# ChrisTho23/DrakeGPT

Hardware: NVIDIA B200
Metric: train_tokens_per_sec_TransformerLM_scaled (higher is better)
Workload: dtype bf16

## Files before the change

drakegpt_b200/csrc/attn_tc.cu:

```cuda
#include <cuda.h>

#include "common.cuh"
#include "ptx.cuh"

namespace dgpt {

using namespace ptx;

int make_tmap_bf16_2d(CUtensorMap* map, const void* base, int64_t inner, int64_t outer, int64_t ld, int box_outer);

static constexpr int HD = 64;
static constexpr int QT = 128;
static constexpr float kLog2e = 1.4426950408889634f;

struct AttnTcP {
  void *o, *dq, *dk, *dv;
  const void *o_in, *d_o;
  float* lse;
  int64_t o_rs, dq_rs, dk_rs, dv_rs, do_rs;
  int B, NH, T;
  float scale, inv_keep;
  uint32_t thr, site;
  uint64_t seed;
  const uint64_t* seed_dev;
};

__device__ __forceinline__ uint32_t pack_bf16(float a, float b) {
  __nv_bfloat162 v = __floats2bfloat162_rn(a, b);
  return *reinterpret_cast<uint32_t*>(&v);
}

__device__ __forceinline__ void store_row32_sw128(uint8_t* tile_base, int row, int c0, const float (&v)[32]) {
  uint8_t* blk = tile_base + (c0 >> 6) * 16384 + row * 128;
  const int chunk0 = (c0 & 63) >> 3;
#pragma unroll
  for (int j = 0; j < 4; ++j) {
    uint4 w;
    w.x = pack_bf16(v[8 * j], v[8 * j + 1]);
    w.y = pack_bf16(v[8 * j + 2], v[8 * j + 3]);
    w.z = pack_bf16(v[8 * j + 4], v[8 * j + 5]);
    w.w = pack_bf16(v[8 * j + 6], v[8 * j + 7]);
    *reinterpret_cast<uint4*>(blk + (((chunk0 + j) ^ (row & 7)) << 4)) = w;
  }
}

static constexpr int kFwd2Threads = 320;
static constexpr int kFwd2QK = 49152;
static constexpr int kFwd2Smem = 2 * kFwd2QK + 2 * 32768 + 256 + 1024;
static constexpr int kWHeavy = 5, kWLight = 2;

struct FwdSched {
  int nheavy, nlight;
  unsigned long long* probe;
};

__global__ void __launch_bounds__(kFwd2Threads, 1)
attn_fwd_tc2_kernel(const __grid_constant__ CUtensorMap map_q32, const __grid_constant__ CUtensorMap map_k,
                    const __grid_constant__ CUtensorMap map_v, AttnTcP p, FwdSched sc) {
  extern __shared__ uint8_t smem_raw[];
  uint8_t* smem = reinterpret_cast<uint8_t*>((reinterpret_cast<uintptr_t>(smem_raw) + 1023) & ~(uintptr_t)1023);
  uint8_t* sQK = smem;
  uint8_t* sV = smem + 2 * kFwd2QK;
  uint64_t* bars = reinterpret_cast<uint64_t*>(sV + 2 * 32768);
  uint64_t *qk_full = bars, *qk_empty = bars + 2, *v_full = bars + 4, *v_empty = bars + 6, *s_full = bars + 8,
           *p_full = bars + 10, *o_full = bars + 12, *slot_free = bars + 14;
  uint32_t* tmem_slot = reinterpret_cast<uint32_t*>(bars + 16);

  clock_probe_begin(sc.probe);
  const int warp = threadIdx.x >> 5, lane = threadIdx.x & 31;
  const int ntile = p.T / QT;

  const int G = gridDim.x, c = blockIdx.x;
  const int hq = sc.nheavy / G, hr = sc.nheavy % G;
  const int nh_c = hq + (c < hr ? 1 : 0);
  const int U = (kWHeavy * sc.nheavy + kWLight * sc.nlight + G - 1) / G;
  const int cap_hi = max(0, (U - kWHeavy * (hq + 1)) / kWLight), cap_lo = max(0, (U - kWHeavy * hq) / kWLight);
  const int cap_total = hr * cap_hi + (G - hr) * cap_lo;
  const int l_start = c < hr ? c * cap_hi : hr * cap_hi + (c - hr) * cap_lo;
  const int l0 = min(sc.nlight, l_start), l1 = min(sc.nlight, l_start + (c < hr ? cap_hi : cap_lo));
  const int n_extra = cap_total < sc.nlight ? (sc.nlight - cap_total - c + G - 1) / G : 0;
  const int n_items = nh_c + (l1 - l0) + max(0, n_extra);
  auto item = [&](int n, int& bh, int& qt) {
    if (n < nh_c) {
      const int hi = c + n * G;
      bh = hi; qt = ntile - 1;
    } else {
      const int m = n - nh_c;
      const int li = m < l1 - l0 ? l0 + m : cap_total + c + (m - (l1 - l0)) * G;
      bh = li; qt = 0;
    }
  };

  if (threadIdx.x == 0) {
    prefetch_tensormap(&map_q32);
    prefetch_tensormap(&map_k);
    prefetch_tensormap(&map_v);
    for (int g = 0; g < 2; ++g) {
      mbar_init(&qk_full[g], 1);
      mbar_init(&qk_empty[g], 1);
      mbar_init(&v_full[g], 1);
      mbar_init(&v_empty[g], 1);
      mbar_init(&s_full[g], 1);
      mbar_init(&p_full[g], 4);
      mbar_init(&o_full[g], 1);
      mbar_init(&slot_free[g], 4);
    }
    fence_barrier_init();
  }
  if (warp == 9) tmem_alloc<512>(tmem_slot);
  tc_fence_before();
  __syncthreads();
  tc_fence_after();
  const uint32_t tmem = *tmem_slot;
  pdl_grid_sync();

  if (warp == 8) {
    for (int n = 0; n < n_items; ++n) {
      const int g = n & 1, k = n >> 1;
      int bh, qt;
      item(n, bh, qt);
      const int nkv = qt + 1, b = bh / p.NH, h = bh % p.NH, row0 = b * p.T;
      uint8_t* q_s = sQK + g * kFwd2QK;
      uint8_t* v_s = sV + g * 32768;
      mbar_wait(&qk_empty[g], (k & 1) ^ 1);
      if (elect_one()) {
        mbar_expect_tx(&qk_full[g], 16384 * (1 + nkv));
        for (int qb = 0; qb < 4; ++qb)
          tma_load_2d(q_s + qb * 4096, &map_q32, &qk_full[g], h * HD, row0 + qt * QT + (g ? 3 - qb : qb) * 32);
        for (int j = 0; j < nkv; ++j) tma_load_2d(q_s + 16384 * (1 + j), &map_k, &qk_full[g], h * HD, row0 + j * QT);
      }
      __syncwarp();
      mbar_wait(&v_empty[g], (k & 1) ^ 1);
      if (elect_one()) {
        mbar_expect_tx(&v_full[g], 16384 * nkv);
        for (int kb = 0; kb < 2 * nkv; ++kb) tma_load_2d(v_s + kb * 8192, &map_v, &v_full[g], h * HD, row0 + kb * 64);
      }
      __syncwarp();
    }
  } else if (warp == 9) {
    constexpr uint32_t idesc_s = make_idesc_bf16(128, 128, 0, 0);
    constexpr uint32_t idesc_o = make_idesc_bf16(128, 64, 0, 1);
    int next_s = 0, next_pv = 0;
    while (next_pv < n_items) {
      bool progressed = false;
      if (next_s < n_items) {
        const int g = next_s & 1, k = next_s >> 1;
        if (mbar_test(&qk_full[g], k & 1) && mbar_test(&slot_free[g], (k & 1) ^ 1)) {
          tc_fence_after();
          int bh, qt;
          item(next_s, bh, qt);
          const int nkv = qt + 1;
          const uint64_t dq0 = make_smem_desc_sw128(smem_u32(sQK + g * kFwd2QK), 16, 1024);
          const uint64_t dk0 = make_smem_desc_sw128(smem_u32(sQK + g * kFwd2QK + 16384), 16, 1024);
          if (elect_one()) {
            for (int j = 0; j < nkv; ++j) {
#pragma unroll
              for (int kk = 0; kk < 4; ++kk)
                tc_mma_bf16(tmem + g * 256 + j * 128, dq0 + (uint64_t)(kk * 2), dk0 + (uint64_t)(j * 1024 + kk * 2), idesc_s, kk > 0);
            }
            tc_commit(&s_full[g]);
            tc_commit(&qk_empty[g]);
          }
          __syncwarp();
          ++next_s;
          progressed = true;
        }
      }
      if (next_pv < next_s) {
        const int g = next_pv & 1, k = next_pv >> 1;
        if (mbar_test(&p_full[g], k & 1) && mbar_test(&v_full[g], k & 1)) {
          tc_fence_after();
          int bh, qt;
          item(next_pv, bh, qt);
          const int nkv = qt + 1;
          const uint64_t dv0 = make_smem_desc_sw128(smem_u32(sV + g * 32768), 8192, 1024);
          if (elect_one()) {
            for (int kb = 0; kb < 2 * nkv; ++kb) {
#pragma unroll
              for (int kk = 0; kk < 4; ++kk)
                tc_mma_bf16_ts(tmem + g * 256 + nkv * 64, tmem + g * 256 + kb * 32 + kk * 8, dv0 + (uint64_t)(kb * 512 + kk * 128),
                               idesc_o, (kb | kk) > 0);
            }
            tc_commit(&o_full[g]);
            tc_commit(&v_empty[g]);
          }
          __syncwarp();
          ++next_pv;
          progressed = true;
        }
      }
      if (!progressed) __nanosleep(32);
    }
  } else {
    const int g = warp >> 2;
    const int quad = warp & 3;
    const int rblk = g ? 3 - quad : quad;
    const int row = rblk * 32 + lane;
    const uint32_t taddr = tmem + (uint32_t)(g * 256) + ((uint32_t)(quad * 32) << 16);
    uint64_t seed = p.seed;
    if (p.thr && p.seed_dev) seed += *p.seed_dev;
    const float sc2 = p.scale * kLog2e;
    for (int n = g; n < n_items; n += 2) {
      const int k = n >> 1;
      int bh, qt;
      item(n, bh, qt);
      const int nkv = qt + 1, b = bh / p.NH, h = bh % p.NH, row0 = b * p.T;
      const int qg = qt * QT + row;
      const int ncols = nkv * QT;
#define FTS(i) do { if (sc.probe && blockIdx.x == 0 && warp == 0 && lane == 0 && k < 3) sc.probe[4 + k * 8 + (i)] = (unsigned long long)clock64(); } while (0)
      FTS(0);
      mbar_wait(&s_full[g], k & 1);
      FTS(1);
      tc_fence_after();
      const int qg_max = qt * QT + rblk * 32 + 31, qg_min = qt * QT + rblk * 32;
      float mx = -INFINITY;
      for (int cc = 0; cc < ncols && cc <= qg_max; cc += 32) {
        uint32_t r[32];
        tmem_ld32(taddr + cc, r);
        tmem_ld_wait();
        if (cc + 31 <= qg_min) {
#pragma unroll
          for (int j = 0; j < 32; ++j) mx = fmaxf(mx, __uint_as_float(r[j]));
        } else {
#pragma unroll
          for (int j = 0; j < 32; ++j)
            if (cc + j <= qg) mx = fmaxf(mx, __uint_as_float(r[j]));
        }
      }
      FTS(2);
      const float msc = mx * sc2;
      float sum = 0.f;
      const uint64_t base = (((uint64_t)b * p.NH + h) * p.T + qg) * (uint64_t)p.T;
      for (int cc = 0; cc < ncols; cc += 32) {
        float e[32];
        if (cc > qg_max) {
#pragma unroll
          for (int j = 0; j < 32; ++j) e[j] = 0.f;
        } else {
          uint32_t r[32];
          tmem_ld32(taddr + cc, r);
          tmem_ld_wait();
          if (cc + 31 <= qg_min) {
#pragma unroll
            for (int j = 0; j < 32; ++j) {
              const float v = exp2f(__uint_as_float(r[j]) * sc2 - msc);
              sum += v;
              e[j] = v;
            }
          } else {
#pragma unroll
            for (int j = 0; j < 32; ++j) {
              const float v = (cc + j <= qg) ? exp2f(__uint_as_float(r[j]) * sc2 - msc) : 0.f;
              sum += v;
              e[j] = v;
            }
          }
          if (p.thr) {
            const DropGroup dg = dropout_group(seed, p.site, (base + cc) >> 5);
#pragma unroll
            for (int j = 0; j < 32; ++j)
              if (dropout_word(dg, j) < p.thr) e[j] = 0.f;
          }
        }
        uint32_t pk[16];
#pragma unroll
        for (int j = 0; j < 16; ++j) pk[j] = pack_bf16(e[2 * j], e[2 * j + 1]);
        tmem_st16(taddr + (cc >> 1), pk);
      }
      if (p.lse) p.lse[((int64_t)b * p.NH + h) * p.T + qg] = mx * p.scale + logf(sum);
      tmem_st_wait();
      tc_fence_before();
      __syncwarp();
      if (lane == 0) mbar_arrive(&p_full[g]);
      FTS(3);
      mbar_wait(&o_full[g], k & 1);
      FTS(4);
      tc_fence_after();
      const float oscale = p.inv_keep / sum;
      __nv_bfloat16* orow = reinterpret_cast<__nv_bfloat16*>(p.o) + (int64_t)(row0 + qg) * p.o_rs + h * HD;
#pragma unroll
      for (int cc = 0; cc < HD; cc += 32) {
        uint32_t r[32];
        tmem_ld32(taddr + nkv * 64 + cc, r);
        tmem_ld_wait();
#pragma unroll
        for (int j = 0; j < 4; ++j) {
          uint4 w;
          w.x = pack_bf16(__uint_as_float(r[8 * j]) * oscale, __uint_as_float(r[8 * j + 1]) * oscale);
          w.y = pack_bf16(__uint_as_float(r[8 * j + 2]) * oscale, __uint_as_float(r[8 * j + 3]) * oscale);
          w.z = pack_bf16(__uint_as_float(r[8 * j + 4]) * oscale, __uint_as_float(r[8 * j + 5]) * oscale);
          w.w = pack_bf16(__uint_as_float(r[8 * j + 6]) * oscale, __uint_as_float(r[8 * j + 7]) * oscale);
          *reinterpret_cast<uint4*>(orow + cc + 8 * j) = w;
        }
      }
      tc_fence_before();
      __syncwarp();
      if (lane == 0) mbar_arrive(&slot_free[g]);
      FTS(5);
    }
  }
  tc_fence_before();
  __syncthreads();
  if (warp == 9) {
    tc_fence_after();
    tmem_dealloc<512>(tmem);
  }
  clock_probe_end(sc.probe);
}

#ifdef DGPT_ATTN_TS
__device__ long long g_attn_ts[64];
#endif
static constexpr int kBwdThreads = 64 + 256;
static constexpr int kBwdSmem = 8 * 16384 + 2 * 32768 + 16384 + 2048 + 1024 + 128;

template <bool DIAG, bool DROP>
__device__ __forceinline__ void bwd_chunk_math(const AttnTcP& p, uint32_t lane_addr_st, uint32_t lane_addr_dp, int row, int k0,
                                               float sc, float lse2, float Dq, uint64_t seed, uint64_t base,
                                               float (&pd)[32], float (&ds)[32]) {
  uint32_t st[32], dp[32];
  tmem_ld32(lane_addr_st + k0, st);
  tmem_ld32(lane_addr_dp + k0, dp);
  tmem_ld_wait();
  DropGroup g = {0u, 0u};
  if (DROP) g = dropout_group(seed, p.site, (base + k0) >> 5);
#pragma unroll
  for (int t = 0; t < 32; ++t) {
    float pv = exp2f(__uint_as_float(st[t]) * sc - lse2);
    if (DIAG) pv = (k0 + t) <= row ? pv : 0.f;
    float dpv = __uint_as_float(dp[t]);
    float pdv = pv;
    if (DROP) {
      const bool keep = dropout_word(g, t) >= p.thr;
      dpv = keep ? dpv * p.inv_keep : 0.f;
      pdv = keep ? pv * p.inv_keep : 0.f;
    }
    pd[t] = pdv;
    ds[t] = pv * (dpv - Dq) * p.scale;
  }
}

template <bool DROP>
__global__ void __launch_bounds__(kBwdThreads, 1)
attn_bwd_tc_kernel(const __grid_constant__ CUtensorMap map_q, const __grid_constant__ CUtensorMap map_k,
                   const __grid_constant__ CUtensorMap map_v, const __grid_constant__ CUtensorMap map_do,
                   const __grid_constant__ CUtensorMap map_o, const __grid_constant__ CUtensorMap map_dq,
                   const __grid_constant__ CUtensorMap map_dk, const __grid_constant__ CUtensorMap map_dv, AttnTcP p) {
  extern __shared__ __align__(1024) uint8_t smem[];
  uint8_t* sQ = smem;
  uint8_t* sK = smem + 2 * 16384;
  uint8_t* sV = smem + 4 * 16384;
  uint8_t* sG = smem + 6 * 16384;
  uint8_t* sPd = smem + 8 * 16384;
  uint8_t* sDs = sPd + 32768;
  uint8_t* sSt = sDs + 32768;
  float* lse_s = reinterpret_cast<float*>(sSt + 16384);
  float* D_s = lse_s + 256;
  uint64_t* bars = reinterpret_cast<uint64_t*>(D_s + 256);
  uint64_t *ld_a = bars, *st_full = bars + 1, *ps_full = bars + 2, *drained = bars + 3, *acc_done = bars + 4;
  uint64_t *ld_b = bars + 5, *ld_c = bars + 6;
  uint64_t* acc_free = bars + 7;
  uint32_t* tmem_slot = reinterpret_cast<uint32_t*>(bars + 8);

  const int warp = threadIdx.x >> 5, lane = threadIdx.x & 31;
#ifdef DGPT_ATTN_TS
#define BTS(i) do { if (blockIdx.x == 0 && blockIdx.y == (gridDim.y / 2) && warp == 2 && lane == 0) g_attn_ts[i] = clock64(); } while (0)
#else
#define BTS(i) do { } while (0)
#endif
  BTS(0);
  const int h = blockIdx.x, b = blockIdx.y;
  const int ntile = p.T / QT;
  const int npair = ntile == 1 ? 1 : 3;
  const int row0 = b * p.T;

  if (threadIdx.x == 0) {
    prefetch_tensormap(&map_q);
    prefetch_tensormap(&map_k);
    prefetch_tensormap(&map_v);
    prefetch_tensormap(&map_do);
    prefetch_tensormap(&map_o);
    mbar_init(ld_a, 1);
    mbar_init(ld_b, 1);
    mbar_init(ld_c, 1);
    mbar_init(st_full, 1);
    mbar_init(ps_full, 8);
    mbar_init(drained, 8);
    mbar_init(acc_done, 1);
    mbar_init(acc_free, 1);
    fence_barrier_init();
  }
  if (warp == 0) {
    __syncwarp();
    pdl_grid_sync();
    if (elect_one()) {
      mbar_expect_tx(ld_a, 16384 * 5);
      tma_load_2d(sG, &map_do, ld_a, h * HD, row0);
      tma_load_2d(sPd, &map_o, ld_a, h * HD, row0);
      tma_load_2d(sQ, &map_q, ld_a, h * HD, row0);
      tma_load_2d(sK, &map_k, ld_a, h * HD, row0);
      tma_load_2d(sV, &map_v, ld_a, h * HD, row0);
      if (ntile > 1) {
        mbar_expect_tx(ld_b, 16384 * 3);
        tma_load_2d(sG + 16384, &map_do, ld_b, h * HD, row0 + QT);
        tma_load_2d(sSt, &map_o, ld_b, h * HD, row0 + QT);
        tma_load_2d(sQ + 16384, &map_q, ld_b, h * HD, row0 + QT);
        mbar_expect_tx(ld_c, 16384 * 2);
        tma_load_2d(sK + 16384, &map_k, ld_c, h * HD, row0 + QT);
        tma_load_2d(sV + 16384, &map_v, ld_c, h * HD, row0 + QT);
      }
    }
  }
  if (warp == 1) tmem_alloc<512>(tmem_slot);
  tc_fence_before();
  __syncthreads();
  tc_fence_after();
  const uint32_t tmem = *tmem_slot;
  constexpr uint32_t TM_ST = 0, TM_DP = 128, TM_DV = 256, TM_DK = 320, TM_DQ = 384;
  if (warp != 0) pdl_grid_sync();

  if (warp == 0) {
  } else if (warp == 1) {
    constexpr uint32_t id_kk = make_idesc_bf16(128, 128, 0, 0);
    constexpr uint32_t id_kmn = make_idesc_bf16(128, 64, 0, 1);
    constexpr uint32_t id_mnmn = make_idesc_bf16(128, 64, 1, 1);
    mbar_wait(ld_a, 0);
    tc_fence_after();
    const uint64_t kQ = make_smem_desc_sw128(smem_u32(sQ), 16, 1024), kK = make_smem_desc_sw128(smem_u32(sK), 16, 1024);
    const uint64_t kV = make_smem_desc_sw128(smem_u32(sV), 16, 1024), kG = make_smem_desc_sw128(smem_u32(sG), 16, 1024);
    const uint64_t kDs = make_smem_desc_sw128(smem_u32(sDs), 16, 1024);
    const uint64_t mQ = make_smem_desc_sw128(smem_u32(sQ), 8192, 1024), mK = make_smem_desc_sw128(smem_u32(sK), 8192, 1024);
    const uint64_t mG = make_smem_desc_sw128(smem_u32(sG), 8192, 1024);
    const uint64_t mPd = make_smem_desc_sw128(smem_u32(sPd), 16384, 1024), mDs = make_smem_desc_sw128(smem_u32(sDs), 16384, 1024);
    auto issue_s_dp = [&](int pr) {
      const int i = pr == 0 ? 0 : 1, j = pr == 2 ? 1 : 0;
      if (elect_one()) {
#pragma unroll
        for (int k = 0; k < 4; ++k)
          tc_mma_bf16(tmem + TM_ST, kQ + (uint64_t)(i * 1024 + k * 2), kK + (uint64_t)(j * 1024 + k * 2), id_kk, k > 0);
#pragma unroll
        for (int k = 0; k < 4; ++k)
          tc_mma_bf16(tmem + TM_DP, kG + (uint64_t)(i * 1024 + k * 2), kV + (uint64_t)(j * 1024 + k * 2), id_kk, k > 0);
        tc_commit(st_full);
      }
      __syncwarp();
    };
    issue_s_dp(0);
    for (int pr = 0; pr < npair; ++pr) {
      const int i = pr == 0 ? 0 : 1, j = pr == 2 ? 1 : 0;
      mbar_wait(ps_full, pr & 1);
      if (pr + 1 < npair) {
        mbar_wait(pr + 1 == 1 ? ld_b : ld_c, 0);
        tc_fence_after();
        issue_s_dp(pr + 1);
      }
      if (pr > 0) mbar_wait(drained, (pr - 1) & 1);
      tc_fence_after();
      const uint32_t acc_vk = (pr == 1) ? 1u : 0u;
      const uint32_t acc_q = (pr == 2) ? 1u : 0u;
      if (elect_one()) {
#pragma unroll
        for (int k = 0; k < 8; ++k)
          tc_mma_bf16(tmem + TM_DV, mPd + (uint64_t)(k * 128), mG + (uint64_t)(i * 1024 + k * 128), id_mnmn, acc_vk | (k > 0));
#pragma unroll
        for (int k = 0; k < 8; ++k)
          tc_mma_bf16(tmem + TM_DK, mDs + (uint64_t)(k * 128), mQ + (uint64_t)(i * 1024 + k * 128), id_mnmn, acc_vk | (k > 0));
#pragma unroll
        for (int k = 0; k < 8; ++k)
          tc_mma_bf16(tmem + TM_DQ, kDs + (uint64_t)((k >> 2) * 1024 + (k & 3) * 2), mK + (uint64_t)(j * 1024 + k * 128), id_kmn,
                      acc_q | (k > 0));
        tc_commit(acc_free);
        if (pr == npair - 1) tc_commit(acc_done);
      }
      __syncwarp();
    }
  } else {
    const int cw = warp - 2;
    const int quad = warp & 3;
    const int half = cw >> 2;
    const int rowl = quad * 32 + lane;
    const int ct = threadIdx.x - 64;
    const uint32_t lane_addr = tmem + ((uint32_t)(quad * 32) << 16);
    uint64_t seed = p.seed;
    if (DROP && p.seed_dev) seed += *p.seed_dev;
    if (ct < p.T) lse_s[ct] = p.lse[((int64_t)b * p.NH + h) * p.T + ct] * kLog2e;
    auto compute_D = [&](int tl, const uint8_t* o_tile) {
      if (ct < QT) {
        const int r = ct;
        const uint8_t* gr = sG + tl * 16384 + r * 128;
        const uint8_t* orow = o_tile + r * 128;
        float acc = 0.f;
#pragma unroll
        for (int c = 0; c < 8; ++c) {
          const int off = (c ^ (r & 7)) << 4;
          const uint4 g = *reinterpret_cast<const uint4*>(gr + off), o = *reinterpret_cast<const uint4*>(orow + off);
          const uint32_t gw[4] = {g.x, g.y, g.z, g.w}, ow[4] = {o.x, o.y, o.z, o.w};
#pragma unroll
          for (int t = 0; t < 4; ++t) {
            const float2 gf = __bfloat1622float2(*reinterpret_cast<const __nv_bfloat162*>(&gw[t]));
            const float2 of = __bfloat1622float2(*reinterpret_cast<const __nv_bfloat162*>(&ow[t]));
            acc = fmaf(gf.x, of.x, acc);
            acc = fmaf(gf.y, of.y, acc);
          }
        }
        D_s[tl * QT + r] = acc;
      }
      asm volatile("bar.sync 1, 256;" ::: "memory");
    };
    BTS(1);
    mbar_wait(ld_a, 0);
    BTS(2);
    compute_D(0, sPd);
    const float sc = p.scale * kLog2e;
    int n_stores = 0;

    auto drain = [&](uint32_t tm_col, const CUtensorMap* map, int tile) {
      uint32_t r[32];
      tmem_ld32(lane_addr + tm_col + half * 32, r);
      if (n_stores > 0) {
        if (ct == 0) bulk_wait_read<0>();
        asm volatile("bar.sync 1, 256;" ::: "memory");
      }
      tmem_ld_wait();
      uint8_t* rp = sSt + rowl * 128;
#pragma unroll
      for (int j = 0; j < 4; ++j) {
        uint4 w;
        w.x = pack_bf16(__uint_as_float(r[8 * j]), __uint_as_float(r[8 * j + 1]));
        w.y = pack_bf16(__uint_as_float(r[8 * j + 2]), __uint_as_float(r[8 * j + 3]));
        w.z = pack_bf16(__uint_as_float(r[8 * j + 4]), __uint_as_float(r[8 * j + 5]));
        w.w = pack_bf16(__uint_as_float(r[8 * j + 6]), __uint_as_float(r[8 * j + 7]));
        *reinterpret_cast<uint4*>(rp + (((half * 4 + j) ^ (rowl & 7)) << 4)) = w;
      }
      fence_proxy_async();
      asm volatile("bar.sync 1, 256;" ::: "memory");
      if (ct == 0) {
        tma_store_2d(map, sSt, h * HD, row0 + tile * QT);
        bulk_commit();
      }
      ++n_stores;
    };

    BTS(3);
    for (int pr = 0; pr < npair; ++pr) {
      const int i = pr == 0 ? 0 : 1, j = pr == 2 ? 1 : 0;
      if (pr == 1) {
        mbar_wait(ld_b, 0);
        compute_D(1, sSt);
      }
      BTS(4 + 4 * pr);
      mbar_wait(st_full, pr & 1);
      BTS(5 + 4 * pr);
      tc_fence_after();
      const int qi = i * QT + rowl;
      const float lse2 = lse_s[qi], Dq = D_s[qi];
      const uint64_t base = (((uint64_t)b * p.NH + h) * p.T + qi) * (uint64_t)p.T + (uint64_t)(j * QT);
      float pd[32], ds[32];
      if (i == j) bwd_chunk_math<true, DROP>(p, lane_addr + TM_ST, lane_addr + TM_DP, rowl, half * 64, sc, lse2, Dq, seed, base, pd, ds);
      else bwd_chunk_math<false, DROP>(p, lane_addr + TM_ST, lane_addr + TM_DP, rowl, half * 64, sc, lse2, Dq, seed, base, pd, ds);
      if (pr > 0) {
        mbar_wait(acc_free, (pr - 1) & 1);
        tc_fence_after();
        if (pr == 1) {
          drain(TM_DQ, &map_dq, 0);
        } else {
          drain(TM_DV, &map_dv, 0);
          drain(TM_DK, &map_dk, 0);
        }
        tc_fence_before();
        __syncwarp();
        if (lane == 0) mbar_arrive(drained);
      }
      BTS(6 + 4 * pr);
      store_row32_sw128(sPd, rowl, half * 64, pd);
      store_row32_sw128(sDs, rowl, half * 64, ds);
      if (i == j) bwd_chunk_math<true, DROP>(p, lane_addr + TM_ST, lane_addr + TM_DP, rowl, half * 64 + 32, sc, lse2, Dq, seed, base, pd, ds);
      else bwd_chunk_math<false, DROP>(p, lane_addr + TM_ST, lane_addr + TM_DP, rowl, half * 64 + 32, sc, lse2, Dq, seed, base, pd, ds);
      store_row32_sw128(sPd, rowl, half * 64 + 32, pd);
      store_row32_sw128(sDs, rowl, half * 64 + 32, ds);
      fence_proxy_async();
      tc_fence_before();
      __syncwarp();
      if (lane == 0) mbar_arrive(ps_full);
      BTS(7 + 4 * pr);
    }
    BTS(16);
    mbar_wait(acc_done, 0);
    BTS(17);
    tc_fence_after();
    const int last = ntile - 1;
    {
      if (n_stores > 0) {
        if (ct == 0) bulk_wait_read<0>();
        asm volatile("bar.sync 1, 256;" ::: "memory");
      }
      uint8_t* tiles[3] = {sPd, sDs, sSt};
      const uint32_t cols[3] = {TM_DV, TM_DK, TM_DQ};
#pragma unroll
      for (int q = 0; q < 3; ++q) {
        uint32_t r[32];
        tmem_ld32(lane_addr + cols[q] + half * 32, r);
        tmem_ld_wait();
        uint8_t* rp = tiles[q] + rowl * 128;
#pragma unroll
        for (int j = 0; j < 4; ++j) {
          uint4 w;
          w.x = pack_bf16(__uint_as_float(r[8 * j]), __uint_as_float(r[8 * j + 1]));
          w.y = pack_bf16(__uint_as_float(r[8 * j + 2]), __uint_as_float(r[8 * j + 3]));
          w.z = pack_bf16(__uint_as_float(r[8 * j + 4]), __uint_as_float(r[8 * j + 5]));
          w.w = pack_bf16(__uint_as_float(r[8 * j + 6]), __uint_as_float(r[8 * j + 7]));
          *reinterpret_cast<uint4*>(rp + (((half * 4 + j) ^ (rowl & 7)) << 4)) = w;
        }
      }
      fence_proxy_async();
      asm volatile("bar.sync 1, 256;" ::: "memory");
      if (ct == 0) {
        tma_store_2d(&map_dv, sPd, h * HD, row0 + last * QT);
        tma_store_2d(&map_dk, sDs, h * HD, row0 + last * QT);
        tma_store_2d(&map_dq, sSt, h * HD, row0 + last * QT);
        bulk_commit();
      }
    }
    if (ct == 0) bulk_wait<0>();
    BTS(18);
  }
  tc_fence_before();
  __syncthreads();
  if (warp == 1) {
    tc_fence_after();
    tmem_dealloc<512>(tmem);
  }
}

bool attn_tc_supported(const dgpt_attn_args* a) {
  if (a->dtype != DGPT_BF16 || a->H != HD || a->Tq != a->Tk) return false;
  if (a->Tk != 128 && a->Tk != 256) return false;
  const int64_t T = a->Tk;
  auto ok = [&](const void* ptr, int64_t bs, int64_t rs) {
    return ptr && ((uintptr_t)ptr & 15) == 0 && rs % 8 == 0 && bs == T * rs;
  };
  if (!ok(a->q, a->q_bs, a->q_rs) || !ok(a->k, a->k_bs, a->k_rs) || !ok(a->v, a->v_bs, a->v_rs) ||
      !ok(a->o, a->o_bs, a->o_rs))
    return false;
  if (a->d_o) {
    if (!ok(a->d_o, a->do_bs, a->do_rs) || !ok(a->dq, a->dq_bs, a->dq_rs) || !ok(a->dk, a->dk_bs, a->dk_rs) ||
        !ok(a->dv, a->dv_bs, a->dv_rs) || !a->lse)
      return false;
  }
  return true;
}

static AttnTcP make_tc_params(const dgpt_attn_args* a) {
  AttnTcP p;
  p.o = a->o; p.dq = a->dq; p.dk = a->dk; p.dv = a->dv; p.o_in = a->o; p.d_o = a->d_o; p.lse = a->lse;
  p.o_rs = a->o_rs; p.dq_rs = a->dq_rs; p.dk_rs = a->dk_rs; p.dv_rs = a->dv_rs; p.do_rs = a->do_rs;
  p.B = a->B; p.NH = a->NH; p.T = a->Tk;
  p.scale = a->scale; p.inv_keep = 1.f / (1.f - a->dropout_p);
  p.thr = dropout_threshold(a->dropout_p); p.site = a->site; p.seed = a->seed; p.seed_dev = a->seed_dev;
  return p;
}

int launch_attn_fwd_tc(const dgpt_attn_args* a, cudaStream_t st) {
  CUtensorMap mq, mk, mv;
  const int64_t rows = (int64_t)a->B * a->Tk, cols = (int64_t)a->NH * HD;
  int rc;
  if ((rc = make_tmap_bf16_2d(&mq, a->q, cols, rows, a->q_rs, 32))) return rc;
  if ((rc = make_tmap_bf16_2d(&mk, a->k, cols, rows, a->k_rs, QT))) return rc;
  if ((rc = make_tmap_bf16_2d(&mv, a->v, cols, rows, a->v_rs, 64))) return rc;
  AttnTcP p = make_tc_params(a);
  static bool attr = false;
  if (!attr) {
    cudaError_t e = cudaFuncSetAttribute(attn_fwd_tc2_kernel, cudaFuncAttributeMaxDynamicSharedMemorySize, kFwd2Smem);
    if (e != cudaSuccess) { set_error("attn_fwd_tc2: smem attribute: %s", cudaGetErrorString(e)); return DGPT_E_LAUNCH; }
    attr = true;
  }
  const int ntile = a->Tk / QT, bh = a->B * a->NH;
  FwdSched sc;
  sc.nheavy = ntile > 1 ? bh : 0;
  sc.nlight = bh;
  sc.probe = clock_probe_buffer();
  int sms = dgpt_sm_count();
  if (sms <= 0) sms = 148;
  const int grid = min(sms, sc.nheavy + sc.nlight);
  launch_pdl(attn_fwd_tc2_kernel, dim3(grid), dim3(kFwd2Threads), kFwd2Smem, st, mq, mk, mv, p, sc);
  return check_launch("attn_fwd_tc2");
}

int launch_attn_bwd_tc(const dgpt_attn_args* a, cudaStream_t st) {
  CUtensorMap mq, mk, mv, mg, mo, mdq, mdk, mdv;
  const int64_t rows = (int64_t)a->B * a->Tk, cols = (int64_t)a->NH * HD;
  int rc;
  if ((rc = make_tmap_bf16_2d(&mq, a->q, cols, rows, a->q_rs, QT))) return rc;
  if ((rc = make_tmap_bf16_2d(&mk, a->k, cols, rows, a->k_rs, QT))) return rc;
  if ((rc = make_tmap_bf16_2d(&mv, a->v, cols, rows, a->v_rs, QT))) return rc;
  if ((rc = make_tmap_bf16_2d(&mg, a->d_o, cols, rows, a->do_rs, QT))) return rc;
  if ((rc = make_tmap_bf16_2d(&mo, a->o, cols, rows, a->o_rs, QT))) return rc;
  if ((rc = make_tmap_bf16_2d(&mdq, a->dq, cols, rows, a->dq_rs, QT))) return rc;
  if ((rc = make_tmap_bf16_2d(&mdk, a->dk, cols, rows, a->dk_rs, QT))) return rc;
  if ((rc = make_tmap_bf16_2d(&mdv, a->dv, cols, rows, a->dv_rs, QT))) return rc;
  static bool attr = false;
  if (!attr) {
    cudaError_t e = cudaFuncSetAttribute(attn_bwd_tc_kernel<true>, cudaFuncAttributeMaxDynamicSharedMemorySize, kBwdSmem);
    if (e == cudaSuccess)
      e = cudaFuncSetAttribute(attn_bwd_tc_kernel<false>, cudaFuncAttributeMaxDynamicSharedMemorySize, kBwdSmem);
    if (e != cudaSuccess) { set_error("attn_bwd_tc: smem attribute: %s", cudaGetErrorString(e)); return DGPT_E_LAUNCH; }
    attr = true;
  }
  AttnTcP p = make_tc_params(a);
  dim3 grid(a->NH, a->B);
  if (p.thr) launch_pdl(attn_bwd_tc_kernel<true>, grid, dim3(kBwdThreads), kBwdSmem, st, mq, mk, mv, mg, mo, mdq, mdk, mdv, p);
  else launch_pdl(attn_bwd_tc_kernel<false>, grid, dim3(kBwdThreads), kBwdSmem, st, mq, mk, mv, mg, mo, mdq, mdk, mdv, p);
#ifdef DGPT_ATTN_TS
  {
    cudaStreamSynchronize(st);
    long long h[64];
    cudaMemcpyFromSymbol(h, g_attn_ts, sizeof(h));
    printf("attn bwd CTA: setup %lld | load wait %lld | D %lld |", h[1] - h[0], h[2] - h[1], h[3] - h[2]);
    for (int pr = 0; pr < 3; ++pr)
      printf(" pair%d: S/dP wait %lld, drains %lld, chunks %lld |", pr, h[5 + 4 * pr] - h[4 + 4 * pr], h[6 + 4 * pr] - h[5 + 4 * pr],
             h[7 + 4 * pr] - h[6 + 4 * pr]);
    printf(" acc wait %lld | final drains %lld | total %lld\n", h[17] - h[16], h[18] - h[17], h[18] - h[0]);
    fflush(stdout);
  }
#endif
  return check_launch("attn_bwd_tc");
}

}
```

Measured before the change: 7.875 million.

## Make attention backward kernel persistent with stats warps computing D and LSE

Converts the attention backward kernel from one CTA per (head, batch) into a persistent grid sized to the SM count, where each CTA loops over work items. The loader warp prefetches the next item's Q/K/V/dO tiles while the current item's MMAs and drains finish, using phase-tracked mbarriers. Two new warps compute the D = rowsum(dO·O) and scaled LSE values straight from global memory into double-buffered shared memory, so the O tile is no longer loaded via TMA and the compute warps skip the D pass. This adds barrier complexity and per-item global loads of O and dO by the stats warps.

```diff
diff --git a/drakegpt_b200/csrc/attn_tc.cu b/drakegpt_b200/csrc/attn_tc.cu
--- a/drakegpt_b200/csrc/attn_tc.cu
+++ b/drakegpt_b200/csrc/attn_tc.cu
@@ -310,9 +310,18 @@
 
 #ifdef DGPT_ATTN_TS
 __device__ long long g_attn_ts[64];
+__device__ unsigned long long g_attn_span[2 * 1024];
 #endif
-static constexpr int kBwdThreads = 64 + 256;
-static constexpr int kBwdSmem = 8 * 16384 + 2 * 32768 + 16384 + 2048 + 1024 + 128;
+static constexpr int kBwdThreads = 64 + 256 + 64;
+static constexpr int kBwdSmem = 8 * 16384 + 2 * 32768 + 16384 + 4096 + 1024 + 128;
+
+struct Phases {
+  uint32_t bits = 0;
+  __device__ __forceinline__ void wait(uint64_t* bars, int k) {
+    mbar_wait(bars + k, (bits >> k) & 1);
+    bits ^= 1u << k;
+  }
+};
 
 template <bool DIAG, bool DROP>
 __device__ __forceinline__ void bwd_chunk_math(const AttnTcP& p, uint32_t lane_addr_st, uint32_t lane_addr_dp, int row, int k0,
@@ -324,10 +333,11 @@
   tmem_ld_wait();
   DropGroup g = {0u, 0u};
   if (DROP) g = dropout_group(seed, p.site, (base + k0) >> 5);
+  const int tmax = row - k0;
 #pragma unroll
   for (int t = 0; t < 32; ++t) {
     float pv = exp2f(__uint_as_float(st[t]) * sc - lse2);
-    if (DIAG) pv = (k0 + t) <= row ? pv : 0.f;
+    if (DIAG) pv = t <= tmax ? pv : 0.f;
     float dpv = __uint_as_float(dp[t]);
     float pdv = pv;
     if (DROP) {
@@ -340,12 +350,25 @@
   }
 }
 
+__device__ __forceinline__ void store_drain_row(uint8_t* tile, int rowl, int half, const uint32_t (&r)[32]) {
+  uint8_t* rp = tile + rowl * 128;
+#pragma unroll
+  for (int j = 0; j < 4; ++j) {
+    uint4 w;
+    w.x = pack_bf16(__uint_as_float(r[8 * j]), __uint_as_float(r[8 * j + 1]));
+    w.y = pack_bf16(__uint_as_float(r[8 * j + 2]), __uint_as_float(r[8 * j + 3]));
+    w.z = pack_bf16(__uint_as_float(r[8 * j + 4]), __uint_as_float(r[8 * j + 5]));
+    w.w = pack_bf16(__uint_as_float(r[8 * j + 6]), __uint_as_float(r[8 * j + 7]));
+    *reinterpret_cast<uint4*>(rp + (((half * 4 + j) ^ (rowl & 7)) << 4)) = w;
+  }
+}
+
 template <bool DROP>
 __global__ void __launch_bounds__(kBwdThreads, 1)
 attn_bwd_tc_kernel(const __grid_constant__ CUtensorMap map_q, const __grid_constant__ CUtensorMap map_k,
                    const __grid_constant__ CUtensorMap map_v, const __grid_constant__ CUtensorMap map_do,
-                   const __grid_constant__ CUtensorMap map_o, const __grid_constant__ CUtensorMap map_dq,
-                   const __grid_constant__ CUtensorMap map_dk, const __grid_constant__ CUtensorMap map_dv, AttnTcP p) {
+                   const __grid_constant__ CUtensorMap map_dq, const __grid_constant__ CUtensorMap map_dk,
+                   const __grid_constant__ CUtensorMap map_dv, AttnTcP p) {
   extern __shared__ __align__(1024) uint8_t smem[];
   uint8_t* sQ = smem;
   uint8_t* sK = smem + 2 * 16384;
@@ -355,31 +378,35 @@
   uint8_t* sDs = sPd + 32768;
   uint8_t* sSt = sDs + 32768;
   float* lse_s = reinterpret_cast<float*>(sSt + 16384);
-  float* D_s = lse_s + 256;
-  uint64_t* bars = reinterpret_cast<uint64_t*>(D_s + 256);
-  uint64_t *ld_a = bars, *st_full = bars + 1, *ps_full = bars + 2, *drained = bars + 3, *acc_done = bars + 4;
-  uint64_t *ld_b = bars + 5, *ld_c = bars + 6;
-  uint64_t* acc_free = bars + 7;
-  uint32_t* tmem_slot = reinterpret_cast<uint32_t*>(bars + 8);
+  float* D_s = lse_s + 512;
+  uint64_t* bars = reinterpret_cast<uint64_t*>(D_s + 512);
+  enum { LD_A, LD_B, LD_C, ST_FULL, PS_FULL, DRAINED, ACC_DONE, ACC_FREE, A_FREE, STATS_FULL, STATS_FREE = STATS_FULL + 2,
+         NBAR = STATS_FREE + 2 };
+  uint64_t *ld_a = bars + LD_A, *ld_b = bars + LD_B, *ld_c = bars + LD_C, *st_full = bars + ST_FULL, *ps_full = bars + PS_FULL;
+  uint64_t *drained = bars + DRAINED, *acc_done = bars + ACC_DONE, *acc_free = bars + ACC_FREE, *a_free = bars + A_FREE;
+  uint32_t* tmem_slot = reinterpret_cast<uint32_t*>(bars + NBAR);
 
   const int warp = threadIdx.x >> 5, lane = threadIdx.x & 31;
 #ifdef DGPT_ATTN_TS
-#define BTS(i) do { if (blockIdx.x == 0 && blockIdx.y == (gridDim.y / 2) && warp == 2 && lane == 0) g_attn_ts[i] = clock64(); } while (0)
+#define BTS(i) do { if (blockIdx.x == 0 && warp == 2 && lane == 0 && (i) < 64) g_attn_ts[i] = clock64(); } while (0)
 #else
 #define BTS(i) do { } while (0)
 #endif
   BTS(0);
-  const int h = blockIdx.x, b = blockIdx.y;
+#ifdef DGPT_ATTN_TS
+  if (threadIdx.x == 64 && blockIdx.x < 1024) g_attn_span[2 * blockIdx.x] = global_timer_ns();
+#endif
   const int ntile = p.T / QT;
   const int npair = ntile == 1 ? 1 : 3;
-  const int row0 = b * p.T;
+  const int a_pair = npair == 1 ? 0 : 1;
+  const int G = gridDim.x;
+  const int n_items = (p.B * p.NH - (int)blockIdx.x + G - 1) / G;
 
   if (threadIdx.x == 0) {
     prefetch_tensormap(&map_q);
     prefetch_tensormap(&map_k);
     prefetch_tensormap(&map_v);
     prefetch_tensormap(&map_do);
-    prefetch_tensormap(&map_o);
     mbar_init(ld_a, 1);
     mbar_init(ld_b, 1);
     mbar_init(ld_c, 1);
@@ -388,28 +415,12 @@
     mbar_init(drained, 8);
     mbar_init(acc_done, 1);
     mbar_init(acc_free, 1);
+    mbar_init(a_free, 1);
+    for (int b = 0; b < 2; ++b) {
+      mbar_init(bars + STATS_FULL + b, 2);
+      mbar_init(bars + STATS_FREE + b, 8);
+    }
     fence_barrier_init();
-  }
-  if (warp == 0) {
-    __syncwarp();
-    pdl_grid_sync();
-    if (elect_one()) {
-      mbar_expect_tx(ld_a, 16384 * 5);
-      tma_load_2d(sG, &map_do, ld_a, h * HD, row0);
-      tma_load_2d(sPd, &map_o, ld_a, h * HD, row0);
-      tma_load_2d(sQ, &map_q, ld_a, h * HD, row0);
-      tma_load_2d(sK, &map_k, ld_a, h * HD, row0);
-      tma_load_2d(sV, &map_v, ld_a, h * HD, row0);
-      if (ntile > 1) {
-        mbar_expect_tx(ld_b, 16384 * 3);
-        tma_load_2d(sG + 16384, &map_do, ld_b, h * HD, row0 + QT);
-        tma_load_2d(sSt, &map_o, ld_b, h * HD, row0 + QT);
-        tma_load_2d(sQ + 16384, &map_q, ld_b, h * HD, row0 + QT);
-        mbar_expect_tx(ld_c, 16384 * 2);
-        tma_load_2d(sK + 16384, &map_k, ld_c, h * HD, row0 + QT);
-        tma_load_2d(sV + 16384, &map_v, ld_c, h * HD, row0 + QT);
-      }
-    }
   }
   if (warp == 1) tmem_alloc<512>(tmem_slot);
   tc_fence_before();
@@ -417,15 +428,38 @@
   tc_fence_after();
   const uint32_t tmem = *tmem_slot;
   constexpr uint32_t TM_ST = 0, TM_DP = 128, TM_DV = 256, TM_DK = 320, TM_DQ = 384;
-  if (warp != 0) pdl_grid_sync();
+  pdl_grid_sync();
 
   if (warp == 0) {
+    Phases ph;
+    for (int it = 0; it < n_items; ++it) {
+      const int bh = blockIdx.x + it * G, h = bh % p.NH, row0 = (bh / p.NH) * p.T;
+      if (it > 0) ph.wait(bars, A_FREE);
+      if (elect_one()) {
+        mbar_expect_tx(ld_a, 16384 * 4);
+        tma_load_2d(sG, &map_do, ld_a, h * HD, row0);
+        tma_load_2d(sQ, &map_q, ld_a, h * HD, row0);
+        tma_load_2d(sK, &map_k, ld_a, h * HD, row0);
+        tma_load_2d(sV, &map_v, ld_a, h * HD, row0);
+      }
+      __syncwarp();
+      if (ntile > 1) {
+        if (it > 0) ph.wait(bars, ACC_DONE);
+        if (elect_one()) {
+          mbar_expect_tx(ld_b, 16384 * 2);
+          tma_load_2d(sG + 16384, &map_do, ld_b, h * HD, row0 + QT);
+          tma_load_2d(sQ + 16384, &map_q, ld_b, h * HD, row0 + QT);
+          mbar_expect_tx(ld_c, 16384 * 2);
+          tma_load_2d(sK + 16384, &map_k, ld_c, h * HD, row0 + QT);
+          tma_load_2d(sV + 16384, &map_v, ld_c, h * HD, row0 + QT);
+        }
+        __syncwarp();
+      }
+    }
   } else if (warp == 1) {
     constexpr uint32_t id_kk = make_idesc_bf16(128, 128, 0, 0);
     constexpr uint32_t id_kmn = make_idesc_bf16(128, 64, 0, 1);
     constexpr uint32_t id_mnmn = make_idesc_bf16(128, 64, 1, 1);
-    mbar_wait(ld_a, 0);
-    tc_fence_after();
     const uint64_t kQ = make_smem_desc_sw128(smem_u32(sQ), 16, 1024), kK = make_smem_desc_sw128(smem_u32(sK), 16, 1024);
     const uint64_t kV = make_smem_desc_sw128(smem_u32(sV), 16, 1024), kG = make_smem_desc_sw128(smem_u32(sG), 16, 1024);
     const uint64_t kDs = make_smem_desc_sw128(smem_u32(sDs), 16, 1024);
@@ -434,6 +468,7 @@
     const uint64_t mPd = make_smem_desc_sw128(smem_u32(sPd), 16384, 1024), mDs = make_smem_desc_sw128(smem_u32(sDs), 16384, 1024);
     auto issue_s_dp = [&](int pr) {
       const int i = pr == 0 ? 0 : 1, j = pr == 2 ? 1 : 0;
+      tc_fence_after();
       if (elect_one()) {
 #pragma unroll
         for (int k = 0; k < 4; ++k)
@@ -445,34 +480,79 @@
       }
       __syncwarp();
     };
+    Phases ph;
+    ph.wait(bars, LD_A);
     issue_s_dp(0);
-    for (int pr = 0; pr < npair; ++pr) {
-      const int i = pr == 0 ? 0 : 1, j = pr == 2 ? 1 : 0;
-      mbar_wait(ps_full, pr & 1);
-      if (pr + 1 < npair) {
-        mbar_wait(pr + 1 == 1 ? ld_b : ld_c, 0);
+    for (int it = 0; it < n_items; ++it) {
+      for (int pr = 0; pr < npair; ++pr) {
+        const int i = pr == 0 ? 0 : 1, j = pr == 2 ? 1 : 0;
+        ph.wait(bars, PS_FULL);
+        if (pr + 1 < npair) {
+          if (pr + 1 == 1) ph.wait(bars, LD_B);
+          else ph.wait(bars, LD_C);
+          issue_s_dp(pr + 1);
+        }
+        if (pr > 0 || it > 0) ph.wait(bars, DRAINED);
         tc_fence_after();
-        issue_s_dp(pr + 1);
-      }
-      if (pr > 0) mbar_wait(drained, (pr - 1) & 1);
-      tc_fence_after();
-      const uint32_t acc_vk = (pr == 1) ? 1u : 0u;
-      const uint32_t acc_q = (pr == 2) ? 1u : 0u;
-      if (elect_one()) {
-#pragma unroll
-        for (int k = 0; k < 8; ++k)
-          tc_mma_bf16(tmem + TM_DV, mPd + (uint64_t)(k * 128), mG + (uint64_t)(i * 1024 + k * 128), id_mnmn, acc_vk | (k > 0));
-#pragma unroll
-        for (int k = 0; k < 8; ++k)
-          tc_mma_bf16(tmem + TM_DK, mDs + (uint64_t)(k * 128), mQ + (uint64_t)(i * 1024 + k * 128), id_mnmn, acc_vk | (k > 0));
-#pragma unroll
-        for (int k = 0; k < 8; ++k)
-          tc_mma_bf16(tmem + TM_DQ, kDs + (uint64_t)((k >> 2) * 1024 + (k & 3) * 2), mK + (uint64_t)(j * 1024 + k * 128), id_kmn,
-                      acc_q | (k > 0));
-        tc_commit(acc_free);
-        if (pr == npair - 1) tc_commit(acc_done);
+        const uint32_t acc_vk = (pr == 1) ? 1u : 0u;
+        const uint32_t acc_q = (pr == 2) ? 1u : 0u;
+        if (elect_one()) {
+#pragma unroll
+          for (int k = 0; k < 8; ++k)
+            tc_mma_bf16(tmem + TM_DV, mPd + (uint64_t)(k * 128), mG + (uint64_t)(i * 1024 + k * 128), id_mnmn, acc_vk | (k > 0));
+#pragma unroll
+          for (int k = 0; k < 8; ++k)
+            tc_mma_bf16(tmem + TM_DK, mDs + (uint64_t)(k * 128), mQ + (uint64_t)(i * 1024 + k * 128), id_mnmn, acc_vk | (k > 0));
+#pragma unroll
+          for (int k = 0; k < 8; ++k)
+            tc_mma_bf16(tmem + TM_DQ, kDs + (uint64_t)((k >> 2) * 1024 + (k & 3) * 2), mK + (uint64_t)(j * 1024 + k * 128), id_kmn,
+                        acc_q | (k > 0));
+          if (pr == npair - 1) tc_commit(acc_done);
+          else tc_commit(acc_free);
+          if (pr == a_pair) tc_commit(a_free);
+        }
+        __syncwarp();
+      }
+      if (it + 1 < n_items) {
+        ph.wait(bars, LD_A);
+        issue_s_dp(0);
+      }
+    }
+  } else if (warp >= 10) {
+    const int st = threadIdx.x - 320;
+    Phases ph;
+    for (int it = 0; it < n_items; ++it) {
+      const int bh = blockIdx.x + it * G, buf = it & 1;
+      if (it >= 2) ph.wait(bars, STATS_FREE + buf);
+      const int64_t r0 = (int64_t)(bh / p.NH) * p.T;
+      const int col = (bh % p.NH) * HD;
+      for (int row = st; row < p.T; row += 64) {
+        const uint4* gr = reinterpret_cast<const uint4*>(reinterpret_cast<const __nv_bfloat16*>(p.d_o) + (r0 + row) * p.do_rs + col);
+        const uint4* orow = reinterpret_cast<const uint4*>(reinterpret_cast<const __nv_bfloat16*>(p.o_in) + (r0 + row) * p.o_rs + col);
+        uint4 gv[8], ov[8];
+#pragma unroll
+        for (int c = 0; c < 8; ++c) {
+          gv[c] = __ldg(gr + c);
+          ov[c] = __ldg(orow + c);
+        }
+        const float lse = p.lse[(int64_t)bh * p.T + row];
+        float acc = 0.f;
+#pragma unroll
+        for (int c = 0; c < 8; ++c) {
+          const uint32_t gw[4] = {gv[c].x, gv[c].y, gv[c].z, gv[c].w}, ow[4] = {ov[c].x, ov[c].y, ov[c].z, ov[c].w};
+#pragma unroll
+          for (int t = 0; t < 4; ++t) {
+            const float2 gf = __bfloat1622float2(*reinterpret_cast<const __nv_bfloat162*>(&gw[t]));
+            const float2 of = __bfloat1622float2(*reinterpret_cast<const __nv_bfloat162*>(&ow[t]));
+            acc = fmaf(gf.x, of.x, acc);
+            acc = fmaf(gf.y, of.y, acc);
+          }
+        }
+        lse_s[buf * 256 + row] = lse * kLog2e;
+        D_s[buf * 256 + row] = acc;
       }
       __syncwarp();
+      if (lane == 0) mbar_arrive(bars + STATS_FULL + buf);
     }
   } else {
     const int cw = warp - 2;
@@ -483,36 +563,10 @@
     const uint32_t lane_addr = tmem + ((uint32_t)(quad * 32) << 16);
     uint64_t seed = p.seed;
     if (DROP && p.seed_dev) seed += *p.seed_dev;
-    if (ct < p.T) lse_s[ct] = p.lse[((int64_t)b * p.NH + h) * p.T + ct] * kLog2e;
-    auto compute_D = [&](int tl, const uint8_t* o_tile) {
-      if (ct < QT) {
-        const int r = ct;
-        const uint8_t* gr = sG + tl * 16384 + r * 128;
-        const uint8_t* orow = o_tile + r * 128;
-        float acc = 0.f;
-#pragma unroll
-        for (int c = 0; c < 8; ++c) {
-          const int off = (c ^ (r & 7)) << 4;
-          const uint4 g = *reinterpret_cast<const uint4*>(gr + off), o = *reinterpret_cast<const uint4*>(orow + off);
-          const uint32_t gw[4] = {g.x, g.y, g.z, g.w}, ow[4] = {o.x, o.y, o.z, o.w};
-#pragma unroll
-          for (int t = 0; t < 4; ++t) {
-            const float2 gf = __bfloat1622float2(*reinterpret_cast<const __nv_bfloat162*>(&gw[t]));
-            const float2 of = __bfloat1622float2(*reinterpret_cast<const __nv_bfloat162*>(&ow[t]));
-            acc = fmaf(gf.x, of.x, acc);
-            acc = fmaf(gf.y, of.y, acc);
-          }
-        }
-        D_s[tl * QT + r] = acc;
-      }
-      asm volatile("bar.sync 1, 256;" ::: "memory");
-    };
     BTS(1);
-    mbar_wait(ld_a, 0);
-    BTS(2);
-    compute_D(0, sPd);
     const float sc = p.scale * kLog2e;
     int n_stores = 0;
+    int h = 0, row0 = 0;
 
     auto drain = [&](uint32_t tm_col, const CUtensorMap* map, int tile) {
       uint32_t r[32];
@@ -522,16 +576,7 @@
         asm volatile("bar.sync 1, 256;" ::: "memory");
       }
       tmem_ld_wait();
-      uint8_t* rp = sSt + rowl * 128;
-#pragma unroll
-      for (int j = 0; j < 4; ++j) {
-        uint4 w;
-        w.x = pack_bf16(__uint_as_float(r[8 * j]), __uint_as_float(r[8 * j + 1]));
-        w.y = pack_bf16(__uint_as_float(r[8 * j + 2]), __uint_as_float(r[8 * j + 3]));
-        w.z = pack_bf16(__uint_as_float(r[8 * j + 4]), __uint_as_float(r[8 * j + 5]));
-        w.w = pack_bf16(__uint_as_float(r[8 * j + 6]), __uint_as_float(r[8 * j + 7]));
-        *reinterpret_cast<uint4*>(rp + (((half * 4 + j) ^ (rowl & 7)) << 4)) = w;
-      }
+      store_drain_row(sSt, rowl, half, r);
       fence_proxy_async();
       asm volatile("bar.sync 1, 256;" ::: "memory");
       if (ct == 0) {
@@ -541,88 +586,89 @@
       ++n_stores;
     };
 
-    BTS(3);
-    for (int pr = 0; pr < npair; ++pr) {
-      const int i = pr == 0 ? 0 : 1, j = pr == 2 ? 1 : 0;
-      if (pr == 1) {
-        mbar_wait(ld_b, 0);
-        compute_D(1, sSt);
-      }
-      BTS(4 + 4 * pr);
-      mbar_wait(st_full, pr & 1);
-      BTS(5 + 4 * pr);
-      tc_fence_after();
-      const int qi = i * QT + rowl;
-      const float lse2 = lse_s[qi], Dq = D_s[qi];
-      const uint64_t base = (((uint64_t)b * p.NH + h) * p.T + qi) * (uint64_t)p.T + (uint64_t)(j * QT);
-      float pd[32], ds[32];
-      if (i == j) bwd_chunk_math<true, DROP>(p, lane_addr + TM_ST, lane_addr + TM_DP, rowl, half * 64, sc, lse2, Dq, seed, base, pd, ds);
-      else bwd_chunk_math<false, DROP>(p, lane_addr + TM_ST, lane_addr + TM_DP, rowl, half * 64, sc, lse2, Dq, seed, base, pd, ds);
-      if (pr > 0) {
-        mbar_wait(acc_free, (pr - 1) & 1);
+    Phases ph;
+    for (int it = 0; it < n_items; ++it) {
+      const int bh = blockIdx.x + it * G, buf = it & 1;
+      h = bh % p.NH;
+      row0 = (bh / p.NH) * p.T;
+      if (it < 4) BTS(2 + 4 * it);
+      ph.wait(bars, STATS_FULL + buf);
+      for (int pr = 0; pr < npair; ++pr) {
+        const int i = pr == 0 ? 0 : 1, j = pr == 2 ? 1 : 0;
+        ph.wait(bars, ST_FULL);
+        if (pr == 0 && it < 4) BTS(3 + 4 * it);
         tc_fence_after();
-        if (pr == 1) {
-          drain(TM_DQ, &map_dq, 0);
-        } else {
-          drain(TM_DV, &map_dv, 0);
-          drain(TM_DK, &map_dk, 0);
-        }
+        const int qi = i * QT + rowl;
+        const float lse2 = lse_s[buf * 256 + qi], Dq = D_s[buf * 256 + qi];
+        const uint64_t base = ((uint64_t)bh * p.T + qi) * (uint64_t)p.T + (uint64_t)(j * QT);
+        float pd[32], ds[32];
+        if (i == j) bwd_chunk_math<true, DROP>(p, lane_addr + TM_ST, lane_addr + TM_DP, rowl, half * 64, sc, lse2, Dq, seed, base, pd, ds);
+        else bwd_chunk_math<false, DROP>(p, lane_addr + TM_ST, lane_addr + TM_DP, rowl, half * 64, sc, lse2, Dq, seed, base, pd, ds);
+        if (pr > 0) {
+          ph.wait(bars, ACC_FREE);
+          tc_fence_after();
+          if (pr == 1) {
+            drain(TM_DQ, &map_dq, 0);
+          } else {
+            drain(TM_DV, &map_dv, 0);
+            drain(TM_DK, &map_dk, 0);
+          }
+          tc_fence_before();
+          __syncwarp();
+          if (lane == 0) mbar_arrive(drained);
+        } else if (n_stores > 0) {
+          if (ct == 0) bulk_wait_read<0>();
+          asm volatile("bar.sync 1, 256;" ::: "memory");
+        }
+        store_row32_sw128(sPd, rowl, half * 64, pd);
+        store_row32_sw128(sDs, rowl, half * 64, ds);
+        if (i == j) bwd_chunk_math<true, DROP>(p, lane_addr + TM_ST, lane_addr + TM_DP, rowl, half * 64 + 32, sc, lse2, Dq, seed, base, pd, ds);
+        else bwd_chunk_math<false, DROP>(p, lane_addr + TM_ST, lane_addr + TM_DP, rowl, half * 64 + 32, sc, lse2, Dq, seed, base, pd, ds);
+        store_row32_sw128(sPd, rowl, half * 64 + 32, pd);
+        store_row32_sw128(sDs, rowl, half * 64 + 32, ds);
+        fence_proxy_async();
         tc_fence_before();
         __syncwarp();
-        if (lane == 0) mbar_arrive(drained);
-      }
-      BTS(6 + 4 * pr);
-      store_row32_sw128(sPd, rowl, half * 64, pd);
-      store_row32_sw128(sDs, rowl, half * 64, ds);
-      if (i == j) bwd_chunk_math<true, DROP>(p, lane_addr + TM_ST, lane_addr + TM_DP, rowl, half * 64 + 32, sc, lse2, Dq, seed, base, pd, ds);
-      else bwd_chunk_math<false, DROP>(p, lane_addr + TM_ST, lane_addr + TM_DP, rowl, half * 64 + 32, sc, lse2, Dq, seed, base, pd, ds);
-      store_row32_sw128(sPd, rowl, half * 64 + 32, pd);
-      store_row32_sw128(sDs, rowl, half * 64 + 32, ds);
-      fence_proxy_async();
-      tc_fence_before();
-      __syncwarp();
-      if (lane == 0) mbar_arrive(ps_full);
-      BTS(7 + 4 * pr);
-    }
-    BTS(16);
-    mbar_wait(acc_done, 0);
-    BTS(17);
-    tc_fence_after();
-    const int last = ntile - 1;
-    {
+        if (lane == 0) mbar_arrive(ps_full);
+      }
+      if (lane == 0) mbar_arrive(bars + STATS_FREE + buf);
+      if (it < 4) BTS(4 + 4 * it);
+      ph.wait(bars, ACC_DONE);
+      tc_fence_after();
       if (n_stores > 0) {
         if (ct == 0) bulk_wait_read<0>();
         asm volatile("bar.sync 1, 256;" ::: "memory");
       }
-      uint8_t* tiles[3] = {sPd, sDs, sSt};
-      const uint32_t cols[3] = {TM_DV, TM_DK, TM_DQ};
-#pragma unroll
-      for (int q = 0; q < 3; ++q) {
+      auto drain_to = [&](uint32_t tm_col, uint8_t* tile) {
         uint32_t r[32];
-        tmem_ld32(lane_addr + cols[q] + half * 32, r);
+        tmem_ld32(lane_addr + tm_col + half * 32, r);
         tmem_ld_wait();
-        uint8_t* rp = tiles[q] + rowl * 128;
-#pragma unroll
-        for (int j = 0; j < 4; ++j) {
-          uint4 w;
-          w.x = pack_bf16(__uint_as_float(r[8 * j]), __uint_as_float(r[8 * j + 1]));
-          w.y = pack_bf16(__uint_as_float(r[8 * j + 2]), __uint_as_float(r[8 * j + 3]));
-          w.z = pack_bf16(__uint_as_float(r[8 * j + 4]), __uint_as_float(r[8 * j + 5]));
-          w.w = pack_bf16(__uint_as_float(r[8 * j + 6]), __uint_as_float(r[8 * j + 7]));
-          *reinterpret_cast<uint4*>(rp + (((half * 4 + j) ^ (rowl & 7)) << 4)) = w;
-        }
-      }
+        store_drain_row(tile, rowl, half, r);
+      };
+      drain_to(TM_DV, sPd);
+      drain_to(TM_DK, sDs);
+      drain_to(TM_DQ, sSt);
+      tc_fence_before();
+      __syncwarp();
+      if (lane == 0) mbar_arrive(drained);
       fence_proxy_async();
       asm volatile("bar.sync 1, 256;" ::: "memory");
       if (ct == 0) {
-        tma_store_2d(&map_dv, sPd, h * HD, row0 + last * QT);
-        tma_store_2d(&map_dk, sDs, h * HD, row0 + last * QT);
-        tma_store_2d(&map_dq, sSt, h * HD, row0 + last * QT);
+        const int last = row0 + (ntile - 1) * QT;
+        tma_store_2d(&map_dv, sPd, h * HD, last);
+        tma_store_2d(&map_dk, sDs, h * HD, last);
+        tma_store_2d(&map_dq, sSt, h * HD, last);
         bulk_commit();
       }
+      ++n_stores;
+      if (it < 4) BTS(5 + 4 * it);
     }
     if (ct == 0) bulk_wait<0>();
     BTS(18);
+#ifdef DGPT_ATTN_TS
+    if (blockIdx.x == 0 && ct == 0) g_attn_ts[19] = n_items;
+    if (ct == 0 && blockIdx.x < 1024) g_attn_span[2 * blockIdx.x + 1] = global_timer_ns();
+#endif
   }
   tc_fence_before();
   __syncthreads();
@@ -687,14 +733,13 @@
 }
 
 int launch_attn_bwd_tc(const dgpt_attn_args* a, cudaStream_t st) {
-  CUtensorMap mq, mk, mv, mg, mo, mdq, mdk, mdv;
+  CUtensorMap mq, mk, mv, mg, mdq, mdk, mdv;
   const int64_t rows = (int64_t)a->B * a->Tk, cols = (int64_t)a->NH * HD;
   int rc;
   if ((rc = make_tmap_bf16_2d(&mq, a->q, cols, rows, a->q_rs, QT))) return rc;
   if ((rc = make_tmap_bf16_2d(&mk, a->k, cols, rows, a->k_rs, QT))) return rc;
   if ((rc = make_tmap_bf16_2d(&mv, a->v, cols, rows, a->v_rs, QT))) return rc;
   if ((rc = make_tmap_bf16_2d(&mg, a->d_o, cols, rows, a->do_rs, QT))) return rc;
-  if ((rc = make_tmap_bf16_2d(&mo, a->o, cols, rows, a->o_rs, QT))) return rc;
   if ((rc = make_tmap_bf16_2d(&mdq, a->dq, cols, rows, a->dq_rs, QT))) return rc;
   if ((rc = make_tmap_bf16_2d(&mdk, a->dk, cols, rows, a->dk_rs, QT))) return rc;
   if ((rc = make_tmap_bf16_2d(&mdv, a->dv, cols, rows, a->dv_rs, QT))) return rc;
@@ -707,19 +752,35 @@
     attr = true;
   }
   AttnTcP p = make_tc_params(a);
-  dim3 grid(a->NH, a->B);
-  if (p.thr) launch_pdl(attn_bwd_tc_kernel<true>, grid, dim3(kBwdThreads), kBwdSmem, st, mq, mk, mv, mg, mo, mdq, mdk, mdv, p);
-  else launch_pdl(attn_bwd_tc_kernel<false>, grid, dim3(kBwdThreads), kBwdSmem, st, mq, mk, mv, mg, mo, mdq, mdk, mdv, p);
+  int sms = dgpt_sm_count();
+  if (sms <= 0) sms = 148;
+  const dim3 grid(min(sms, a->B * a->NH));
+  if (p.thr) launch_pdl(attn_bwd_tc_kernel<true>, grid, dim3(kBwdThreads), kBwdSmem, st, mq, mk, mv, mg, mdq, mdk, mdv, p);
+  else launch_pdl(attn_bwd_tc_kernel<false>, grid, dim3(kBwdThreads), kBwdSmem, st, mq, mk, mv, mg, mdq, mdk, mdv, p);
 #ifdef DGPT_ATTN_TS
   {
     cudaStreamSynchronize(st);
     long long h[64];
     cudaMemcpyFromSymbol(h, g_attn_ts, sizeof(h));
-    printf("attn bwd CTA: setup %lld | load wait %lld | D %lld |", h[1] - h[0], h[2] - h[1], h[3] - h[2]);
-    for (int pr = 0; pr < 3; ++pr)
-      printf(" pair%d: S/dP wait %lld, drains %lld, chunks %lld |", pr, h[5 + 4 * pr] - h[4 + 4 * pr], h[6 + 4 * pr] - h[5 + 4 * pr],
-             h[7 + 4 * pr] - h[6 + 4 * pr]);
-    printf(" acc wait %lld | final drains %lld | total %lld\n", h[17] - h[16], h[18] - h[17], h[18] - h[0]);
+    const int n = (int)min(h[19], 4LL);
+    printf("attn bwd CTA 0 (%lld items): setup %lld |", h[19], h[1] - h[0]);
+    for (int it = 0; it < n; ++it) {
+      const long long* t = h + 2 + 4 * it;
+      printf(" item%d: S/dP wait %lld, pairs %lld, acc wait + drains %lld, period %lld |", it, t[1] - t[0], t[2] - t[1],
+             t[3] - t[2], (it + 1 < n ? t[4] : t[3]) - t[0]);
+    }
+    printf(" tail %lld | total %lld\n", h[18] - h[2 + 4 * (n - 1) + 3], h[18] - h[0]);
+    static unsigned long long sp[2 * 1024];
+    cudaMemcpyFromSymbol(sp, g_attn_span, sizeof(sp));
+    const int g = (int)min(grid.x, 1024u);
+    unsigned long long t0 = ~0ull, e0 = ~0ull, e1 = 0;
+    for (int c = 0; c < g; ++c) {
+      t0 = std::min(t0, sp[2 * c]);
+      e0 = std::min(e0, sp[2 * c + 1]);
+      e1 = std::max(e1, sp[2 * c + 1]);
+    }
+    printf("attn bwd %d CTAs: first entry -> first / last CTA done %llu / %llu ns; CTA 0 %llu ns (%.0f MHz)\n", g, e0 - t0,
+           e1 - t0, sp[1] - sp[0], (double)(h[18] - h[0]) * 1e3 / (double)(sp[1] - sp[0]));
     fflush(stdout);
   }
 #endif
```

Result: faster. 7.992 million (median of 6 runs) (+1.5%).
